# montyhall/bot7

Measured on AMD Instinct MI355X. Metric: EI candidates scored/sec at N=2048,d=32, higher is better.
Workload: dtype f64

## Files before the change

### bot7_amd/build.py

```python
import concurrent.futures
import os
import subprocess
import sys

HERE = os.path.dirname(os.path.abspath(__file__))
ROOT = os.path.dirname(HERE)
CSRC = os.path.join(HERE, "csrc")
BUILD = os.path.join(HERE, "_build")
OUT = os.path.join(HERE, "libbot7hip.so")
SOURCES = ["context.hip", "grid_api.hip", "gp_api.hip", "nominate.hip", "blr_api.hip", "sobol.hip", "covar.hip", "potrf.hip", "potrf_persist.hip", "posterior.hip", "score.hip", "extras.hip", "comm.hip", "group.hip", "blr_small.hip", "gp_small.hip", "kpost_small.hip", "batch.hip"]
DIAG_ONLY_SOURCES = ["nll_small.hip"]
DIAG_OUT = os.path.join(ROOT, "tools", "_build", "libbot7hip_diag.so")
HEADERS = [os.path.join(CSRC, "b7_internal.h"), os.path.join(CSRC, "gemm_f64.h"), os.path.join(CSRC, "potrf_diag.h"), os.path.join(CSRC, "comm_rccl.h"), os.path.join(CSRC, "ksx_exp.h"), os.path.join(CSRC, "exp_table.h"),
           os.path.join(ROOT, "include", "bot7hip.h")]
HIPCC = os.environ.get("HIPCC", "/opt/rocm/bin/hipcc")
FLAGS = ["-O3", "-std=c++17", "-fPIC", "--offload-arch=gfx950", "-fno-fast-math", "-Wall",
         "-I" + os.path.join(ROOT, "include"), "-I" + CSRC, "-I/opt/rocm/include"]


def _stale(target, deps):
    if not os.path.exists(target):
        return True
    t = os.path.getmtime(target)
    return any(os.path.getmtime(d) > t for d in deps)


EXTRA_FLAGS = {"covar.hip": ["-mllvm", "-amdgpu-mfma-vgpr-form"], "batch.hip": ["-mllvm", "-amdgpu-mfma-vgpr-form"]}


def _compile(src, diag=False):
    obj = os.path.join(BUILD, ("diag_" if diag else "") + src.replace(".hip", ".o"))
    path = os.path.join(CSRC, src)
    if _stale(obj, [path] + HEADERS + [os.path.abspath(__file__)]):
        subprocess.check_call([HIPCC] + FLAGS + EXTRA_FLAGS.get(src, []) + (["-DB7_DIAG"] if diag else []) + ["-c", path, "-o", obj])
        return obj, True
    return obj, False


def _mentions_diag(src):
    return "B7_DIAG" in open(os.path.join(CSRC, src)).read()


def build_diag(verbose=False):
    build()
    os.makedirs(os.path.dirname(DIAG_OUT), exist_ok=True)
    todo = [s for s in SOURCES if _mentions_diag(s)] + DIAG_ONLY_SOURCES
    with concurrent.futures.ThreadPoolExecutor(max_workers=min(8, len(todo))) as ex:
        res = dict(zip(todo, ex.map(lambda s: _compile(s, True), todo)))
    objs = [res[s][0] if s in res else os.path.join(BUILD, s.replace(".hip", ".o")) for s in SOURCES + DIAG_ONLY_SOURCES]
    if any(ch for _, ch in res.values()) or _stale(DIAG_OUT, objs):
        subprocess.check_call([HIPCC, "-shared", "-fPIC", "--offload-arch=gfx950", "-o", DIAG_OUT] + objs +
                              ["-ldl", "-Wl,-rpath,/opt/rocm/lib", "-Wl,--no-undefined", "-Wl,-Bsymbolic"])
        if verbose:
            print("built", DIAG_OUT)
    return DIAG_OUT


def posterior_isa():
    out = os.path.join(BUILD, "posterior.s")
    path = os.path.join(CSRC, "posterior.hip")
    if _stale(out, [path] + HEADERS + [os.path.abspath(__file__)]):
        subprocess.check_call([HIPCC] + [f for f in FLAGS if f != "-fPIC"] + ["-S", "--cuda-device-only", "-Wno-unused-command-line-argument",
                                                                            path, "-o", out])
    return out


def check_agpr_discipline():
    import re
    text = open(posterior_isa()).read()
    found = {}
    for m in re.finditer(r"^(_ZN\S*post_kernel_w4(?:ILi(\d)E|tILi\d+ELi\d+E)\S*):[^\n]*\n(.*?)\n\s*s_endpgm", text, flags=re.S | re.M):
        nj = int(m.group(2)) if m.group(2) else 16
        ntiles = 32 if nj == 16 else 8 * nj
        in_asm, stats, bad = False, {"mfma": 0, "mfma_from_zero": 0, "acc_reads": 0, "scratch": 0}, []
        for line in m.group(3).split("\n"):
            code = line.split(";")[0]
            if "ASMSTART" in line:
                in_asm = True
                continue
            if "ASMEND" in line:
                in_asm = False
                continue
            if in_asm:
                stats["mfma"] += "v_mfma_f64_16x16x4_f64" in code
                stats["mfma_from_zero"] += bool(re.search(r"v_mfma_f64_16x16x4_f64 a\[[^\]]*\], v\[[^\]]*\], v\[[^\]]*\], 0\s*$", code))
                stats["acc_reads"] += "v_accvgpr_read_b32" in code
            else:
                if re.search(r"(?<![A-Za-z0-9_.])a(\[|\d)", code):
                    bad.append(line.strip())
                stats["scratch"] += "scratch_" in code
        if bad or stats["scratch"] or stats["mfma_from_zero"] != ntiles or stats["acc_reads"] != 8 * ntiles:
            raise RuntimeError("post_kernel_w4<%d>: AGPR discipline broken: %r, compiler-generated AGPR uses: %r"
                               % (nj, stats, bad[:5]))
        found[nj] = stats
    if not {2, 4} <= set(found):
        raise RuntimeError("post_kernel_w4<2> and <4> expected in the ISA of posterior.hip, found %r" % sorted(found))
    return found


def build_post_probe():
    src = os.path.join(ROOT, "tools", "post_probe.hip")
    out = os.path.join(ROOT, "tools", "_build", "post_probe")
    os.makedirs(os.path.dirname(out), exist_ok=True)
    if _stale(out, [src, os.path.join(ROOT, "tools", "post_kernel_w8.h"), os.path.join(CSRC, "posterior.hip")] + HEADERS):
        subprocess.check_call([HIPCC, "--offload-arch=gfx950", "-O3", "-std=c++17", "-fno-fast-math", "-Wno-unused-value",
                               "-DB7_POST_NO_LAUNCHERS", "-I" + os.path.join(ROOT, "include"), "-I" + CSRC,
                               "-I/opt/rocm/include", "-o", out, src, "-Wl,-rpath,/opt/rocm/lib"])
    return out


def build(force=False, verbose=False):
    os.makedirs(BUILD, exist_ok=True)
    if force:
        for f in os.listdir(BUILD):
            os.remove(os.path.join(BUILD, f))
    with concurrent.futures.ThreadPoolExecutor(max_workers=min(8, len(SOURCES) + 2)) as ex:
        isa = ex.submit(check_agpr_discipline)
        probe = ex.submit(build_post_probe)
        results = list(ex.map(_compile, SOURCES))
        isa.result()
        probe.result()
    objs = [o for o, _ in results]
    if any(changed for _, changed in results) or _stale(OUT, objs):
        subprocess.check_call([HIPCC, "-shared", "-fPIC", "--offload-arch=gfx950", "-o", OUT] + objs +
                              ["-ldl", "-Wl,-rpath,/opt/rocm/lib", "-Wl,--no-undefined", "-Wl,-Bsymbolic"])
        if verbose:
            print("built", OUT)
    return OUT


if __name__ == "__main__":
    build(force="--force" in sys.argv, verbose=True)
    if "--diag" in sys.argv:
        build_diag(verbose=True)
```

### bot7_amd/csrc/b7_internal.h

```cpp
#pragma once
#include <hip/hip_runtime.h>
#include <stddef.h>
#include <stdint.h>

#include <map>
#include <string>
#include <vector>

#include "bot7hip.h"

constexpr int B7_NPAD = 128;
constexpr int B7_PANEL = 64;
constexpr int B7_PERSIST_NMAX = 4096;
constexpr int B7_MROWS = 256;
constexpr int B7_MAX_D = 96;

constexpr int B7_TAB_VAL = 0;
constexpr int B7_TAB_IDX = 1;
constexpr int B7_TAB_STATUS = 2;
constexpr int B7_TAB_ROWS = 3;
constexpr int B7_TAB_ROW0 = 4;
constexpr int B7_TAB_W = B7_TAB_ROW0 + B7_MAX_D;
constexpr int B7_MAX_WORLD = 64;

static inline int b7_dpad_class(int d) {
  return d <= 4 ? 4 : d <= 8 ? 8 : d <= 16 ? 16 : d <= 32 ? 32 : d <= 48 ? 48 : d <= 64 ? 64 : 96;
}

constexpr size_t B7_INFO_HEAD_BYTES = 16 + sizeof(double) * 257 + 8;
constexpr size_t B7_PERSIST_FLAG_WORDS_MAX = 16 + 2 * 64 * 64 + 2 * 64;
constexpr size_t B7_INFO_BYTES = B7_INFO_HEAD_BYTES + 4 * B7_PERSIST_FLAG_WORDS_MAX;

struct DevBuf {
  void *p = nullptr;
  size_t cap = 0;
};

struct PinBuf {
  void *host = nullptr, *dev = nullptr;
  size_t bytes = 0;
};

struct FitBlock { int info[4]; double terms[257]; };
struct BestPair { double v; int64_t i; };
constexpr int SOBOL_DIMS = 40;
constexpr int SOBOL_BITS = 30;
struct SobolTable {
  uint32_t v[SOBOL_DIMS][SOBOL_BITS];
};

constexpr size_t B7_PINNED_BYTES = 16384;
struct PinnedBlock {
  FitBlock fit;
  alignas(256) BestPair best;
  alignas(4096) double fmin[256];
  alignas(4096) double vec[B7_MAX_D + 3];
};
static_assert(offsetof(PinnedBlock, fit) == 0 && offsetof(PinnedBlock, best) == 2304 && offsetof(PinnedBlock, fmin) == 4096 &&
                  offsetof(PinnedBlock, vec) == 8192 && sizeof(PinnedBlock) <= B7_PINNED_BYTES,
              "pinned block: kernels and copies address these slots");

constexpr size_t B7_SCRATCH_BYTES = 64 * 1024;
struct ScratchBlock {
  double lenscale[256];
  double fmin[256];
  SobolTable sobol;
  double minmax[2 * B7_MAX_D];
  alignas(4096) double colvec[2 * B7_MAX_D];
};
static_assert(offsetof(ScratchBlock, lenscale) == 0 && offsetof(ScratchBlock, fmin) == 2048 && offsetof(ScratchBlock, sobol) == 4096 &&
                  offsetof(ScratchBlock, minmax) == 4096 + sizeof(SobolTable) && offsetof(ScratchBlock, colvec) == 12288 &&
                  sizeof(ScratchBlock) <= B7_SCRATCH_BYTES,
              "scratch block: the layout every earlier build used");

constexpr int B7_ACC_NONE = 0, B7_ACC_LINEAR = 1, B7_ACC_LOG = 2;

struct PhaseStat {
  double ms = 0.0;
  int64_t launches = 0;
};

struct ScoreParams {
  int kind = 0, S = 0, upper = 0;
  const double *mu = nullptr, *var = nullptr, *fmin = nullptr;
  long long stride = 0;
  double fmin0 = 0.0, tradeoff = 0.0, sign = 0.0;
};

struct b7_ctx {
  int device = 0;
  hipStream_t stream = nullptr;
  hipEvent_t ev_fit = nullptr;
  std::string err;
  int cus = 0;

  DevBuf grid[2];
  int grid_cur = 0;
  int64_t M = 0;
  int d = 0;

  bool fitted = false;
  bool have_data = false;
  int model_kind = 0;
  int N = 0, Npad = 0, dfit = 0, dpad = 0, ycols = 0;
  int yld = 1;
  double amp = 0, noise = 0, mean = 0;
  b7_gp_opts opts;
  int kernel = B7_KERNEL_ARDSE;
  DevBuf xobs;
  DevBuf w;
  DevBuf zsc;
  DevBuf zss;
  DevBuf K;
  DevBuf L;
  DevBuf Linv;
  DevBuf W;
  DevBuf dinv;
  DevBuf alpha;
  DevBuf resid;
  DevBuf atmp;
  DevBuf info;
  DevBuf ybuf;

  bool predicted = false;
  int64_t Mpred = 0;
  DevBuf mu;
  DevBuf var;
  DevBuf acc;
  bool acc_valid = false;
  int spin_us = 500;
  bool npad_small = true;
  bool potrf_small = true;
  bool blr_small = true;
  double fmin_scalar = 0.0;
  bool acc_fresh = false;
  int acc_kind = 0;
  DevBuf ks;
  size_t ks_bytes = (size_t)4 << 30;
  int diag_variant = 1;
  int inverse_inline = 1;
  PinnedBlock *pinned = nullptr, *pinned_dev = nullptr;
  std::vector<double> net_host;
  PinBuf pin_blr;
  PinBuf pin_eval;
  PinBuf pin_nll;
  bool fmin_staged = false;
  bool potrf_attrs_set = false;
  bool linv_done = false;
  int potrf_sched = 3;
  int syrk_small = 1;
  int potrf_defer = 1;
  int potrf_group = 2;
  struct JobList { DevBuf buf; int n = 0; };
  std::map<int, JobList> pjobs_cache;
  DevBuf pstamps;
  int pjobs_nb = 0, pjobs_n = 0;
  DevBuf bhyp, bw, bzsc, bzss, bK, bL, bdinv, bflags, binfo, bresid, bterms, bLinv, balpha, bmu, bvar;
  bool persist_attr_set = false, persist_stamps = false;
  int persist_helpers = 0;
  int persist_aborts = 0;
  int nll_small = 1;
  bool kpost_small = true;
  bool fit_small = true;
  int persist_fault = -1;
  int potrf_sched_saved = 0;
  DevBuf part;
  DevBuf ticket;
  DevBuf scratch;
  DevBuf tmpgrid;
  DevBuf tmpmu, tmpvar;
  DevBuf fant;
  DevBuf bel;
  DevBuf belvec;
  PinBuf pin_bel;
  DevBuf feat;
  size_t feat_zeroed_bytes = 0;
  int feat_z = -1;
  int64_t Mfeat = 0;
  int zdim = 0;
  uint64_t feat_version = 0, grid_version = 0;
  DevBuf netbuf;

  void *comm = nullptr;
  int comm_rank = 0, comm_world = 1;
  DevBuf slots;
  uint64_t *tab_host = nullptr;
  uint64_t *tab_host_dev = nullptr;
  struct b7_group *group = nullptr;
  bool group_busy = false;
  bool win_valid = false;
  int64_t win_idx1 = 0;
  int win_rank = -1, win_d = 0;
  double win_row[B7_MAX_D];
  int64_t shard_rows[B7_MAX_WORLD];
  int shard_world = 0;

  hipEvent_t tev[B7_MAX_TIMERS][2];
  bool tev_init = false;
  bool profile = false;
  std::map<std::string, PhaseStat> phases;
  struct PendingPhase { const char *name; hipEvent_t e0, e1; };
  std::vector<PendingPhase> pending;
  std::vector<hipEvent_t> free_events;
  hipEvent_t phase_e0 = nullptr;
};

int b7_fail(b7_ctx *c, int code, const char *fmt, ...);
#define B7_HIP(c, expr)                                                                          \
  do {                                                                                           \
    hipError_t e__ = (expr);                                                                     \
    if (e__ != hipSuccess)                                                                       \
      return b7_fail((c), e__ == hipErrorOutOfMemory ? B7_ERR_NOMEM : B7_ERR_HIP, "%s:%d: %s", \
                     __FILE_NAME__, __LINE__, hipGetErrorString(e__));                           \
  } while (0)
#define B7_TRY(expr)          \
  do {                        \
    int rc__ = (expr);        \
    if (rc__ != B7_OK) return rc__; \
  } while (0)

int b7_ensure(b7_ctx *c, DevBuf &b, size_t bytes);
void b7_release(DevBuf &b);
int b7_pin_ensure(b7_ctx *c, PinBuf &b, size_t bytes, bool mapped);
static inline ScratchBlock *b7_scratch(const b7_ctx *c) { return static_cast<ScratchBlock *>(c->scratch.p); }

struct PhaseScope {
  b7_ctx *c;
  const char *name;
  PhaseScope(b7_ctx *c, const char *name);
  ~PhaseScope();
};

static inline int64_t round_up(int64_t x, int64_t m) { return (x + m - 1) / m * m; }
int npad_of(const b7_ctx *c, int64_t n);

int launch_sobol(b7_ctx *c, double *out, int64_t size, int dims, int64_t skip, const double *mins,
                 const double *maxes);
int launch_random_grid(b7_ctx *c, double *out, int64_t size, int dims, uint64_t seed, int64_t row_offset,
                       const double *mins, const double *maxes);
int launch_remove_row(b7_ctx *c, const double *src, double *dst, int64_t M, int d, int64_t idx0);
int launch_remove_rows(b7_ctx *c, const double *src, double *dst, int64_t M, int d, const int64_t *cuts_dev, int ncut);
int launch_colrange(b7_ctx *c, const double *grid, int64_t M, int d, double *out_dev);
int launch_col_affine(b7_ctx *c, double *grid, int64_t M, int d, const double *v_dev, bool mul);
int launch_gather_rows(b7_ctx *c, const double *src, double *out, const int64_t *idx0_dev, int64_t n, int d);

struct KBatchDesc {
  int64_t s_w = 0, s_zsc = 0, s_zsh = 0, s_out = 0;
  const double *amp = nullptr;
  int64_t s_alpha = 0, s_mu = 0;
  const double *mean = nullptr;
};
struct ObsSet {
  const double *zsc;
  const double *zsh;
  int npad;
  const double *w = nullptr;
  KBatchDesc batch;
};
int launch_prep_obs_aux(b7_ctx *c, const double *xobs, const double *ls_dev, int N, int npad, double *zsc,
                        double *zsh);
int launch_k_generic(b7_ctx *c, const double *xq, int64_t rows, int64_t Mtotal, const ObsSet &o, double *out);
int launch_prep_obs(b7_ctx *c, const double *xobs, const double *lenscale_sq_dev, int N, int d);
int launch_kxx(b7_ctx *c, double diag_add);
int launch_ksx_batch(b7_ctx *c, int S, const double *xq, int64_t rows, int64_t Mtotal, const double *w, const double *zsc,
                     const double *zss, const double *amp_dev, const double *mean_dev, const double *alpha, double *ks,
                     int64_t s_out, double *mu, int64_t s_mu);
int launch_kxx_batch(b7_ctx *c, int B, const double *ls_dev, const double *amp_dev, const double *noise_dev, double *w,
                     double *zsc, double *zss, double *K);
int launch_ksx(b7_ctx *c, const double *xq, int64_t row0, int64_t rows, int64_t Mtotal, int d, double *ks,
               double *mu, int ycols);

struct FactorNote {
  bool alpha_done = false;
  int *report_written = nullptr;
};
int launch_potrf(b7_ctx *c, double extra, bool with_inverse, int *report_hint = nullptr, FactorNote *note = nullptr);
int launch_trtri(b7_ctx *c);
int launch_potrf_persist(b7_ctx *c, double extra, bool with_inverse);
int launch_nll_batch(b7_ctx *c, int B, const double *K, double *L, double *dinv, unsigned *flags, int *info,
                     const double *resid, double *terms);
int launch_nll_one(b7_ctx *c, const double *K, double *L, double *dinv, unsigned *flags, int *info, const double *resid,
                   double *terms, double extra);
size_t persist_flag_words_host(int nb);
int launch_potrf_small(b7_ctx *c, int B, const double *K, double *L, double *Linv, double *dinv, const double *resid, double *alpha,
                       double extra, int *info, int *report_dev, int64_t sK, int64_t sL, int64_t sdinv, int64_t svec, int sinfo);
int launch_blr_head_small(b7_ctx *c, const double *Z, int N, int z, int ldz, const double *yv, double alpha_prec, double beta,
                          int *report_dev);
int launch_blr_heads_small(b7_ctx *c, int S, const double *Z, int N, int z, int ldz, const double *yraw_dev, const double *hyp3_dev,
                           double *L, double *Linv, double *m, double *b, int *info, int *report_dev, double *terms);
int launch_post_heads(b7_ctx *c, int S, const double *Linv, const double *feat, int64_t rows, int64_t Mtotal, double *var, int64_t svar,
                      const double *zero_dev, const double *invbeta_dev);
int launch_gemv_rows_batch(b7_ctx *c, int S, const double *A, int lda, const double *x, int64_t sx, int n, const double *base_dev,
                           int64_t rows, double *y, int64_t sy);
int launch_nll_small(b7_ctx *c, int B, const double *hyp_dev, const double *hyp_host, double *terms_dev, int *info_dev,
                     unsigned *done_dev);
bool kpost_small_applies(const b7_ctx *c);
int launch_kpost_small(b7_ctx *c, int S, const double *xq, int64_t M, const double *w, const double *zsc, const double *zss,
                       const double *Linv, const double *alpha, const double *hyp_dev, double amp, double noise, double mean,
                       double *mu, double *var, int64_t sout);
bool gp_small_applies(const b7_ctx *c);
static inline bool fit_small_applies(const b7_ctx *c) {
  return c->fit_small && c->potrf_sched == 3 && c->inverse_inline && gp_small_applies(c);
}
int launch_nll_small8(b7_ctx *c, int B, const double *hyp_dev, const double *hyp_host, double *terms_dev, int *info_dev,
                      unsigned *done_dev);
int launch_fit_small(b7_ctx *c, int B, const double *hyp_dev, const double *hyp_host, double *hyp_out, double *w, double *zsc,
                     double *zss, double *L, double *Linv, double *dinv, double *alpha, double *resid, int *info_dev,
                     int *report_dev);
int launch_alpha(b7_ctx *c, int *report_dev = nullptr, int report_words = 0, const FactorNote &note = FactorNote());
int launch_alpha_batch(b7_ctx *c, int B, const double *Linv, const double *resid, double *alpha, const int *report_src = nullptr,
                       int *report_dev = nullptr, int report_words = 0);
int launch_fit_batch(b7_ctx *c, int B, const double *K, double *L, double *Linv, double *dinv, unsigned *flags, int *info);
int launch_nll_terms(b7_ctx *c, double *out_dev);
int launch_fro_norm_sq(b7_ctx *c, const double *A, int n, int ld, double *out_dev);
int launch_set_identity(b7_ctx *c);

// ... 137 lines not shown
```

### bot7_amd/csrc/context.hip

```cpp
#include <stdarg.h>
#include <stdio.h>
#include <stdlib.h>
#include <string.h>

#include "b7_internal.h"

static thread_local std::string g_create_err;

int b7_fail(b7_ctx *c, int code, const char *fmt, ...) {
  char buf[512];
  va_list ap;
  va_start(ap, fmt);
  vsnprintf(buf, sizeof(buf), fmt, ap);
  va_end(ap);
  if (c)
    c->err = buf;
  else
    g_create_err = buf;
  return code;
}

int b7_ensure(b7_ctx *c, DevBuf &b, size_t bytes) {
  if (bytes == 0) bytes = 16;
  if (b.cap >= bytes) return B7_OK;
  if (b.p) {
    B7_HIP(c, hipStreamSynchronize(c->stream));
    B7_HIP(c, hipFree(b.p));
    b.p = nullptr;
    b.cap = 0;
  }
  hipError_t e = hipMalloc(&b.p, bytes);
  if (e != hipSuccess) {
    b.p = nullptr;
    return b7_fail(c, B7_ERR_NOMEM, "hipMalloc(%zu bytes): %s", bytes, hipGetErrorString(e));
  }
  b.cap = bytes;
  return B7_OK;
}

void b7_release(DevBuf &b) {
  if (b.p) (void)hipFree(b.p);
  b.p = nullptr;
  b.cap = 0;
}

int b7_pin_ensure(b7_ctx *c, PinBuf &b, size_t bytes, bool mapped) {
  if (b.bytes >= bytes) return B7_OK;
  B7_HIP(c, hipStreamSynchronize(c->stream));
  if (b.host) (void)hipHostFree(b.host);
  b = PinBuf();
  B7_HIP(c, hipHostMalloc(&b.host, 2 * bytes, mapped ? hipHostMallocMapped : hipHostMallocDefault));
  if (mapped) B7_HIP(c, hipHostGetDevicePointer(&b.dev, b.host, 0));
  b.bytes = 2 * bytes;
  return B7_OK;
}

static hipEvent_t phase_event(b7_ctx *c) {
  if (!c->free_events.empty()) {
    hipEvent_t e = c->free_events.back();
    c->free_events.pop_back();
    return e;
  }
  hipEvent_t e = nullptr;
  (void)hipEventCreate(&e);
  return e;
}

static void resolve_phases(b7_ctx *c) {
  if (c->pending.empty()) return;
  (void)hipStreamSynchronize(c->stream);
  for (const b7_ctx::PendingPhase &p : c->pending) {
    float ms = 0.f;
    if (p.e0 && p.e1 && hipEventElapsedTime(&ms, p.e0, p.e1) == hipSuccess) {
      PhaseStat &s = c->phases[p.name];
      s.ms += ms;
      s.launches += 1;
    }
    if (p.e0) c->free_events.push_back(p.e0);
    if (p.e1) c->free_events.push_back(p.e1);
  }
  c->pending.clear();
}

PhaseScope::PhaseScope(b7_ctx *c_, const char *name_) : c(c_), name(name_) {
  if (!c->profile) return;
  c->phase_e0 = phase_event(c);
  if (c->phase_e0) (void)hipEventRecord(c->phase_e0, c->stream);
}
PhaseScope::~PhaseScope() {
  if (!c->profile || !c->phase_e0) return;
  hipEvent_t e1 = phase_event(c);
  if (e1) (void)hipEventRecord(e1, c->stream);
  c->pending.push_back({name, c->phase_e0, e1});
  c->phase_e0 = nullptr;
  if (c->pending.size() >= 4096) resolve_phases(c);
}

int npad_of(const b7_ctx *c, int64_t n) { return (c->npad_small && n <= 64) ? 64 : (int)round_up(n, B7_NPAD); }

static int timers_init(b7_ctx *c) {
  if (c->tev_init) return B7_OK;
  for (int i = 0; i < B7_MAX_TIMERS; ++i) {
    B7_HIP(c, hipEventCreate(&c->tev[i][0]));
    B7_HIP(c, hipEventCreate(&c->tev[i][1]));
  }
  c->tev_init = true;
  return B7_OK;
}

extern "C" {

int b7_abi_version(void) { return B7_ABI_VERSION; }

int b7_create(b7_ctx **out, int device_id) {
  if (!out) return b7_fail(nullptr, B7_ERR_INVALID, "b7_create: out is NULL");
  *out = nullptr;
  int ndev = 0;
  hipError_t e = hipGetDeviceCount(&ndev);
  if (e != hipSuccess || ndev <= 0)
    return b7_fail(nullptr, B7_ERR_HIP, "no HIP device available (%s); libbot7hip has no CPU path",
                   e == hipSuccess ? "device count 0" : hipGetErrorString(e));
  if (device_id < 0 || device_id >= ndev)
    return b7_fail(nullptr, B7_ERR_INVALID, "device_id %d out of range [0,%d)", device_id, ndev);
  e = hipSetDevice(device_id);
  if (e != hipSuccess) return b7_fail(nullptr, B7_ERR_HIP, "hipSetDevice: %s", hipGetErrorString(e));
  hipDeviceProp_t prop;
  e = hipGetDeviceProperties(&prop, device_id);
  if (e != hipSuccess) return b7_fail(nullptr, B7_ERR_HIP, "hipGetDeviceProperties: %s", hipGetErrorString(e));
  if (strncmp(prop.gcnArchName, "gfx950", 6) != 0)
    return b7_fail(nullptr, B7_ERR_UNSUPPORTED, "device %d is %s; libbot7hip is built for gfx950 only", device_id,
                   prop.gcnArchName);
  b7_ctx *c = new b7_ctx();
  c->device = device_id;
  c->cus = prop.multiProcessorCount;
  b7_gp_default_opts(&c->opts);
  if (const char *pv = getenv("B7_SPIN_US")) c->spin_us = atoi(pv);
#ifdef B7_DIAG
  if (const char *pv = getenv("B7_DIAG_VARIANT")) c->diag_variant = atoi(pv);
  if (const char *pv = getenv("B7_NPAD_SMALL")) c->npad_small = atoi(pv) != 0;
  if (const char *pv = getenv("B7_POTRF_SMALL")) c->potrf_small = atoi(pv) != 0;
  if (getenv("B7_POTRF_SCHED") || getenv("B7_DIAG_VARIANT") || getenv("B7_INVERSE_INLINE")) c->potrf_small = c->fit_small = false;
  if (const char *pv = getenv("B7_BLR_SMALL")) c->blr_small = atoi(pv) != 0;
  if (const char *pv = getenv("B7_INVERSE_INLINE")) c->inverse_inline = atoi(pv);
  if (const char *pv = getenv("B7_POTRF_SCHED")) c->potrf_sched = atoi(pv);
  c->persist_stamps = getenv("B7_PERSIST_STAMPS") != nullptr;
  if (const char *pv = getenv("B7_PERSIST_HELPERS")) c->persist_helpers = atoi(pv);
  if (const char *pv = getenv("B7_PERSIST_FAULT")) c->persist_fault = atoi(pv);
  if (const char *pv = getenv("B7_NLL_SMALL")) c->nll_small = atoi(pv);
  if (const char *pv = getenv("B7_FIT_SMALL")) c->fit_small = atoi(pv) != 0;
  if (const char *pv = getenv("B7_KPOST_SMALL")) c->kpost_small = atoi(pv) != 0;
  if (const char *pv = getenv("B7_SYRK_SMALL")) c->syrk_small = atoi(pv) ? 1 : 0;
  if (const char *pv = getenv("B7_POTRF_DEFER")) c->potrf_defer = atoi(pv) ? 1 : 0;
  if (const char *pv = getenv("B7_POTRF_GROUP")) {
    const int g = atoi(pv);
    if (g >= 1 && g <= 8) c->potrf_group = g;
  }
#endif
  e = hipStreamCreateWithFlags(&c->stream, hipStreamNonBlocking);
  if (e == hipSuccess) e = hipEventCreateWithFlags(&c->ev_fit, hipEventDisableTiming);
  if (e == hipSuccess) e = hipHostMalloc((void **)&c->pinned, B7_PINNED_BYTES, hipHostMallocMapped);
  if (e == hipSuccess) e = hipHostGetDevicePointer((void **)&c->pinned_dev, c->pinned, 0);
  if (e != hipSuccess) {
    if (c->pinned) (void)hipHostFree(c->pinned);
    if (c->stream) (void)hipStreamDestroy(c->stream);
    delete c;
    return b7_fail(nullptr, B7_ERR_HIP, "stream / pinned result block creation: %s", hipGetErrorString(e));
  }
  if (b7_ensure(c, c->scratch, B7_SCRATCH_BYTES) != B7_OK) {
    g_create_err = c->err;
    b7_destroy(c);
    return B7_ERR_NOMEM;
  }
  *out = c;
  return B7_OK;
}

void b7_destroy(b7_ctx *c) {
  if (!c) return;
  (void)hipSetDevice(c->device);
  (void)hipStreamSynchronize(c->stream);
  (void)b7_comm_destroy(c);
  DevBuf *all[] = {&c->grid[0], &c->grid[1], &c->xobs, &c->w,     &c->zsc,  &c->zss,     &c->K,      &c->L,
                   &c->Linv,    &c->W,       &c->dinv, &c->alpha, &c->resid, &c->info,   &c->ybuf,   &c->mu,
                   &c->var,     &c->acc,     &c->ks,   &c->part,  &c->scratch, &c->tmpgrid, &c->tmpmu, &c->tmpvar, &c->fant, &c->feat, &c->netbuf, &c->atmp, &c->slots, &c->pstamps,
                   &c->bhyp, &c->bw, &c->bzsc, &c->bzss, &c->bK, &c->bL, &c->bdinv, &c->bflags, &c->binfo, &c->bresid, &c->bterms,
                   &c->bLinv, &c->balpha, &c->bmu, &c->bvar, &c->ticket, &c->bel, &c->belvec};
  for (auto &kv : c->pjobs_cache) b7_release(kv.second.buf);
  for (DevBuf *b : all) b7_release(*b);
  if (c->tev_init)
    for (int i = 0; i < B7_MAX_TIMERS; ++i) {
      (void)hipEventDestroy(c->tev[i][0]);
      (void)hipEventDestroy(c->tev[i][1]);
    }
  resolve_phases(c);
  if (c->pinned) (void)hipHostFree(c->pinned);
  for (PinBuf *b : {&c->pin_eval, &c->pin_blr, &c->pin_nll, &c->pin_bel})
    if (b->host) (void)hipHostFree(b->host);
  if (c->tab_host) (void)hipHostFree(c->tab_host);
  for (hipEvent_t e : c->free_events) (void)hipEventDestroy(e);
  if (c->phase_e0) (void)hipEventDestroy(c->phase_e0);
  if (c->ev_fit) (void)hipEventDestroy(c->ev_fit);
  (void)hipStreamDestroy(c->stream);
  delete c;
}

const char *b7_last_error(const b7_ctx *c) { return c ? c->err.c_str() : g_create_err.c_str(); }

int b7_device_info(b7_ctx *c, char *name_out, int *compute_units, int64_t *hbm_bytes) {
  if (!c) return B7_ERR_INVALID;
  hipDeviceProp_t prop;
  B7_HIP(c, hipGetDeviceProperties(&prop, c->device));
  if (name_out) snprintf(name_out, 64, "%s (%s)", prop.name, prop.gcnArchName);
  if (compute_units) *compute_units = prop.multiProcessorCount;
  if (hbm_bytes) *hbm_bytes = (int64_t)prop.totalGlobalMem;
  return B7_OK;
}

int b7_sync(b7_ctx *c) {
  if (!c) return B7_ERR_INVALID;
  B7_HIP(c, hipStreamSynchronize(c->stream));
  return B7_OK;
}

int b7_set_workspace(b7_ctx *c, int64_t bytes) {
  if (!c || bytes < (int64_t)(8 * 128 * 128)) return c ? b7_fail(c, B7_ERR_INVALID, "workspace too small") : B7_ERR_INVALID;
  c->ks_bytes = (size_t)bytes;
  return B7_OK;
}

int b7_timer_start(b7_ctx *c, int slot) {
  if (!c || slot < 0 || slot >= B7_MAX_TIMERS) return B7_ERR_INVALID;
  B7_TRY(timers_init(c));
  B7_HIP(c, hipEventRecord(c->tev[slot][0], c->stream));
  return B7_OK;
}

int b7_timer_stop(b7_ctx *c, int slot) {
  if (!c || slot < 0 || slot >= B7_MAX_TIMERS) return B7_ERR_INVALID;
  B7_TRY(timers_init(c));
  B7_HIP(c, hipEventRecord(c->tev[slot][1], c->stream));
  return B7_OK;
}

int b7_timer_ms(b7_ctx *c, int slot, float *ms_out) {
  if (!c || slot < 0 || slot >= B7_MAX_TIMERS || !ms_out) return B7_ERR_INVALID;
  B7_TRY(timers_init(c));
  B7_HIP(c, hipEventSynchronize(c->tev[slot][1]));
  B7_HIP(c, hipEventElapsedTime(ms_out, c->tev[slot][0], c->tev[slot][1]));
  return B7_OK;
}

int b7_profile_enable(b7_ctx *c, int on) {
  if (!c) return B7_ERR_INVALID;
  c->profile = on != 0;
  return B7_OK;
}

int b7_profile_reset(b7_ctx *c) {
  if (!c) return B7_ERR_INVALID;
  resolve_phases(c);
  c->phases.clear();
  return B7_OK;
}

int b7_profile_get(b7_ctx *c, const char *phase, double *ms_total, int64_t *launches) {
  if (!c || !phase) return B7_ERR_INVALID;
  resolve_phases(c);
  auto it = c->phases.find(phase);
  if (ms_total) *ms_total = it == c->phases.end() ? 0.0 : it->second.ms;
  if (launches) *launches = it == c->phases.end() ? 0 : it->second.launches;
  return B7_OK;
}

}
```

### bot7_amd/csrc/posterior.hip

```cpp
#include "b7_internal.h"
#include <utility>

#ifdef B7_POST_STAMPS
__device__ unsigned long long b7_post_stamps[4 * 4096];
extern "C" int b7dbg_post_stamps(unsigned long long *out, int nblocks) {
  return (int)hipMemcpyFromSymbol(out, HIP_SYMBOL(b7_post_stamps), sizeof(unsigned long long) * 4 * nblocks);
}
#endif

typedef double d2_t __attribute__((ext_vector_type(2)));

struct PostBatch {
  int64_t sLinv = 0, sks = 0, svar = 0;
  const double *base = nullptr, *var_add = nullptr;
};

namespace w4 {
constexpr int BM = 128, BK = 16, LD = BK + 1, A_DBL = BM * LD;

#define B7_W4_ACC_REGS \
  "a0", "a1", "a2", "a3", "a4", "a5", "a6", "a7", "a8", "a9", "a10", "a11", "a12", "a13", "a14", "a15", \
  "a16", "a17", "a18", "a19", "a20", "a21", "a22", "a23", "a24", "a25", "a26", "a27", "a28", "a29", "a30", \
  "a31", "a32", "a33", "a34", "a35", "a36", "a37", "a38", "a39", "a40", "a41", "a42", "a43", "a44", "a45", \
  "a46", "a47", "a48", "a49", "a50", "a51", "a52", "a53", "a54", "a55", "a56", "a57", "a58", "a59", "a60", \
// ... 292 lines not shown
      mfma_tile<NJ, i, j, ZERO>(use.a[i], use.b[j]);
      static_for<KMAX>([&](auto k_) {
        constexpr int sidx = m * NSIDE / NM + decltype(k_)::value;
        if constexpr (sidx < (m + 1) * NSIDE / NM) side(std::integral_constant<int, sidx>{});
      });
    });
  }

  template <int FIRST, int NEXT_FIRST, bool ZERO>
  static __device__ __forceinline__ void stage(Set &s0, Set &s1, Data &g, double *__restrict__ cur, double *__restrict__ nxt,
                                               int fa, int fb, int wofs, const double *__restrict__ pa,
                                               const double *__restrict__ pb, int64_t lda, Cursor &ld) {
    constexpr int H = NC / 2;
    const double *qa = pa + ((int64_t)ld.t * BMT) * lda + ld.kb * BK, *qb = pb + ld.kb * BK;
    ld.advance();
    kstep<FIRST, ZERO, NP + H>(s0, [&](auto s_) {
      constexpr int x = decltype(s_)::value;
      if constexpr (x < NP) {
        if constexpr (x < NJ || x - NJ >= FIRST) read_one<x, 1>(s1, cur + fa, cur + fb);
      } else {
        store_chunk<x - NP>(g, nxt + wofs);
      }
    });
    kstep<FIRST, false, NP + NC - H>(s1, [&](auto s_) {
      constexpr int x = decltype(s_)::value;
      if constexpr (x < NP) {
        if constexpr (x < NJ || x - NJ >= FIRST) read_one<x, 2>(s0, cur + fa, cur + fb);
      } else {
        store_chunk<H + x - NP>(g, nxt + wofs);
      }
    });
    kstep<FIRST, false, NP + NC>(s0, [&](auto s_) {
      constexpr int x = decltype(s_)::value;
      if constexpr (x < NP) {
        if constexpr (x < NJ || x - NJ >= FIRST) read_one<x, 3>(s1, cur + fa, cur + fb);
      } else {
        load_chunk<x - NP>(g, qa, qb, lda);
      }
    });
    __builtin_amdgcn_s_waitcnt(0xC07F);
    __builtin_amdgcn_s_barrier();
    kstep<FIRST, false, NP>(s1, [&](auto s_) {
      constexpr int x = decltype(s_)::value;
      if constexpr (x < NJ || x - NJ >= NEXT_FIRST) read_one<x, 0>(s0, nxt + fa, nxt + fb);
    });
  }
};

template <int NJ, int NR>
__global__ void __launch_bounds__(256)
    post_kernel_w4t(const double *__restrict__ Linv, const double *__restrict__ ks, int Npad, int64_t row0, int64_t Mtotal,
                    double base, double sgn, double var_add, int clamp, double var_min, double *__restrict__ var,
                    PostBatch bat) {
  using T = Tall<NJ, NR>;
  constexpr int BMT = T::BMT, BN = T::BN, NC = T::NC, NP = T::NP;
  extern __shared__ __align__(16) double sm[];
  if (bat.base) {
    const int64_t y = blockIdx.y;
    Linv += y * bat.sLinv;
    ks += y * bat.sks;
    var += y * bat.svar;
    base = bat.base[y];
    if (bat.var_add) var_add = bat.var_add[y];
  }
  const int lane = threadIdx.x & 63, wave = __builtin_amdgcn_readfirstlane(threadIdx.x >> 6);
#ifdef B7_POST_STAMPS
  const unsigned long long st0 = __builtin_amdgcn_s_memtime(), sr0 = __builtin_amdgcn_s_memrealtime();
  __builtin_amdgcn_s_waitcnt(0xC07F);
#endif
  const int64_t lda = Npad;
  const int r0 = threadIdx.x >> 3, kc = threadIdx.x & 7;
  const double *pa = Linv + (int64_t)r0 * lda + 2 * kc;
  const double *pb = ks + ((int64_t)blockIdx.x * BN + r0) * lda + 2 * kc;
  const int wofs = r0 * LD + 2 * kc;
  const int fa = (lane & 15) * LD + (lane >> 4);
  const int fb = T::A_DBLT + (wave * 16 * NJ + (lane & 15)) * LD + (lane >> 4);

  const int ntiles = Npad / BMT;
  typename T::Cursor ld{0, 0, ntiles};
  typename T::Data g;
  typename T::Set s0, s1;
  double *const b0 = sm, *const b1 = sm + T::STAGE_DBL;
  static_for<NC>([&](auto c_) { T::template load_chunk<decltype(c_)::value>(g, pa, pb, lda); });
  ld.advance();
  static_for<NC>([&](auto c_) { T::template store_chunk<decltype(c_)::value>(g, b0 + wofs); });
  {
    const double *qa = pa + ((int64_t)ld.t * BMT) * lda + ld.kb * BK, *qb = pb + ld.kb * BK;
    static_for<NC>([&](auto c_) { T::template load_chunk<decltype(c_)::value>(g, qa, qb, lda); });
    ld.advance();
  }
  __builtin_amdgcn_s_waitcnt(0xC07F);
  __builtin_amdgcn_s_barrier();
  static_for<NP>([&](auto p_) { T::template read_one<decltype(p_)::value, 0>(s0, b0 + fa, b0 + fb); });

  double colss[2][NJ] = {};
#define B7_STAGE(F, NF, Z, CUR, NXT) T::template stage<F, NF, Z>(s0, s1, g, CUR, NXT, fa, fb, wofs, pa, pb, lda, ld)
  for (int t = 0; t < ntiles; ++t) {
    B7_STAGE(0, 0, true, b0, b1);
    if (t > 0) {
      for (int p = 0; p < (NR / 2) * t - 1; ++p) {
        B7_STAGE(0, 0, false, b1, b0);
        B7_STAGE(0, 0, false, b0, b1);
      }
      B7_STAGE(0, 0, false, b1, b0);
      B7_STAGE(0, 1, false, b0, b1);
    }
    static_for<NR - 1>([&](auto q_) {
      constexpr int Q = decltype(q_)::value + 1;
      if constexpr (Q % 2 == 1)
        B7_STAGE(Q, (Q + 1) % NR, false, b1, b0);
      else
        B7_STAGE(Q, (Q + 1) % NR, false, b0, b1);
    });
    asm volatile("s_nop 15\n\ts_nop 15\n\ts_nop 15" ::: "memory");
    static_for<(NR / 4) * NJ>([&](auto qj_) {
      constexpr int q = decltype(qj_)::value / NJ, j = decltype(qj_)::value % NJ;
      double s = 0.0;
      static_for<4>([&](auto i_) {
        double v[4];
        read_tile<NJ, 4 * q + decltype(i_)::value, j>(v);
#pragma unroll
        for (int r = 0; r < 4; ++r) s = __builtin_fma(v[r], v[r], s);
      });
      colss[q & 1][j] += s;
    });
  }
#undef B7_STAGE

#pragma unroll
  for (int j = 0; j < NJ; ++j) {
    double v0 = colss[0][j], v1 = colss[1][j];
    v0 += __shfl_xor(v0, 16);
    v0 += __shfl_xor(v0, 32);
    v1 += __shfl_xor(v1, 16);
    v1 += __shfl_xor(v1, 32);
    const int64_t gidx = row0 + (int64_t)blockIdx.x * BN + wave * 16 * NJ + j * 16 + lane;
    if (lane < 16 && gidx < Mtotal) {
      double ss = v0;
      ss += v1;
      double v = (base + sgn * ss) + var_add;
      if (clamp) v = (v < var_min) ? var_min : v;
      var[gidx] = v;
    }
  }
#ifdef B7_POST_STAMPS
  if (threadIdx.x == 0 && blockIdx.x < 4096) {
    const unsigned long long st1 = __builtin_amdgcn_s_memtime(), sr1 = __builtin_amdgcn_s_memrealtime();
    __builtin_amdgcn_s_waitcnt(0xC07F);
    unsigned long long *o = b7_post_stamps + 4 * blockIdx.x;
    o[0] = st0, o[1] = sr0, o[2] = st1, o[3] = sr1;
  }
#endif
}
}

namespace small64 {
typedef double d4_t __attribute__((ext_vector_type(4)));
constexpr int NB = 64, LLD = NB + 2, BN = 64;
constexpr int LDS_BYTES = BN * LLD * 8;

__global__ void __launch_bounds__(256)
    post_small_kernel(const double *__restrict__ Linv, const double *__restrict__ ks, int64_t row0, int64_t Mtotal, int ntiles,
                      double base, double sgn, double var_add, int clamp, double var_min, double *__restrict__ var, PostBatch bat) {
  extern __shared__ __align__(16) double sm[];
  if (bat.base) {
    const int64_t y = blockIdx.y;
    Linv += y * bat.sLinv;
    ks += y * bat.sks;
    var += y * bat.svar;
    base = bat.base[y];
    if (bat.var_add) var_add = bat.var_add[y];
  }
  double *Ks = sm;
  const int tid = threadIdx.x, lane = tid & 63, wave = tid >> 6, lr = lane & 15, lq = lane >> 4;
  d2_t pv[BN / 8];
  auto fetch = [&](int tile) {
    const double *kt = ks + ((int64_t)tile * BN) * NB;
#pragma unroll
    for (int i = 0; i < BN / 8; ++i) {
      const int e = tid + 256 * i;
      pv[i] = *reinterpret_cast<const d2_t *>(kt + (int64_t)(e >> 5) * NB + 2 * (e & 31));
    }
  };
  int tile = blockIdx.x;
  if (tile < ntiles) fetch(tile);
  double af[40];
#pragma unroll
  for (int I = 0; I < 4; ++I)
#pragma unroll
    for (int k4 = 0; k4 < 4 * (I + 1); ++k4) af[2 * I * (I + 1) + k4] = Linv[(int64_t)(I * 16 + lr) * NB + 4 * k4 + lq];
#pragma unroll
  for (int g = 0; g < 4; ++g)
    asm volatile("" : "+v"(af[10 * g]), "+v"(af[10 * g + 1]), "+v"(af[10 * g + 2]), "+v"(af[10 * g + 3]), "+v"(af[10 * g + 4]),
                      "+v"(af[10 * g + 5]), "+v"(af[10 * g + 6]), "+v"(af[10 * g + 7]), "+v"(af[10 * g + 8]), "+v"(af[10 * g + 9]));
  for (; tile < ntiles; tile += gridDim.x) {
#pragma unroll
    for (int i = 0; i < BN / 8; ++i) {
      const int e = tid + 256 * i, r = e >> 5, c2 = 2 * (e & 31);
      Ks[r * LLD + c2] = pv[i][0];
      Ks[r * LLD + c2 + 1] = pv[i][1];
    }
    __syncthreads();
    if (tile + (int)gridDim.x < ntiles) fetch(tile + gridDim.x);
    __builtin_amdgcn_sched_barrier(0);
    constexpr int NJ = BN / 64;
    double ss[NJ];
#pragma unroll
    for (int j = 0; j < NJ; ++j) {
      const double *bp = Ks + (wave * 16 * NJ + j * 16 + lr) * LLD + lq;
      double bf[16];
#pragma unroll
      for (int k4 = 0; k4 < 16; ++k4) bf[k4] = bp[4 * k4];
      double s = 0.0;
#pragma unroll
      for (int I = 0; I < 4; ++I) {
        d4_t c = {0.0, 0.0, 0.0, 0.0};
#ifdef B7_PS_ABLATE
        c = __builtin_amdgcn_mfma_f64_16x16x4f64(af[2 * I * (I + 1)], bf[I], c, 0, 0, 0);
#else
#pragma unroll
        for (int k4 = 0; k4 < 4 * (I + 1); ++k4) c = __builtin_amdgcn_mfma_f64_16x16x4f64(af[2 * I * (I + 1) + k4], bf[k4], c, 0, 0, 0);
#endif
#pragma unroll
        for (int r = 0; r < 4; ++r) s = __builtin_fma(c[r], c[r], s);
      }
      ss[j] = s;
    }
#pragma unroll
    for (int j = 0; j < NJ; ++j) {
      double v = ss[j];
      v += __shfl_xor(v, 16);
      v += __shfl_xor(v, 32);
      const int64_t gidx = row0 + (int64_t)tile * BN + wave * 16 * NJ + j * 16 + lr;
      if (lane < 16 && gidx < Mtotal) {
        double o = (base + sgn * v) + var_add;
        if (clamp) o = (o < var_min) ? var_min : o;
        var[gidx] = o;
      }
    }
    __syncthreads();
  }
}
}

#ifndef B7_POST_NO_LAUNCHERS
namespace {
struct PostArgs {
  const double *Linv, *ks;
  double *var;
  double base, sgn, var_add;
  int S;
  PostBatch pb;
};

template <int NJ>
int launch_post_w4(b7_ctx *c, const PostArgs &a, int64_t row0, int64_t rows, int64_t Mtotal) {
  constexpr int lds = w4::lds_bytes<NJ>();
  B7_HIP(c, hipFuncSetAttribute(reinterpret_cast<const void *>(w4::post_kernel_w4<NJ>),
                                hipFuncAttributeMaxDynamicSharedMemorySize, lds));
  hipLaunchKernelGGL(w4::post_kernel_w4<NJ>, dim3((unsigned)(rows / (64 * NJ)), a.S), dim3(256), lds, c->stream, a.Linv, a.ks,
                     c->Npad, row0, Mtotal, a.base, a.sgn, a.var_add, c->opts.var_clamp, c->opts.var_min, a.var, a.pb);
  B7_HIP(c, hipGetLastError());
  return B7_OK;
}

template <int NJ, int NR>
int launch_post_tall(b7_ctx *c, const PostArgs &a, int64_t row0, int64_t rows, int64_t Mtotal) {
  using T = w4::Tall<NJ, NR>;
  auto kern = w4::post_kernel_w4t<NJ, NR>;
  B7_HIP(c, hipFuncSetAttribute(reinterpret_cast<const void *>(kern), hipFuncAttributeMaxDynamicSharedMemorySize,
                                T::LDS_BYTES));
  hipLaunchKernelGGL(kern, dim3((unsigned)(rows / T::BN), a.S), dim3(256), T::LDS_BYTES, c->stream, a.Linv, a.ks, c->Npad, row0,
                     Mtotal, a.base, a.sgn, a.var_add, c->opts.var_clamp, c->opts.var_min, a.var, a.pb);
  B7_HIP(c, hipGetLastError());
  return B7_OK;
}

int launch_post_small(b7_ctx *c, const PostArgs &a, int64_t row0, int64_t rows, int64_t Mtotal) {
  B7_HIP(c, hipFuncSetAttribute(reinterpret_cast<const void *>(small64::post_small_kernel), hipFuncAttributeMaxDynamicSharedMemorySize,
                                small64::LDS_BYTES));
  const int ntiles = (int)(rows / small64::BN), S = a.S > 0 ? a.S : 1;
  int gx = (2 * c->cus + S - 1) / S;
  if (gx > ntiles) gx = ntiles;
  if (gx < 1) gx = 1;
  hipLaunchKernelGGL(small64::post_small_kernel, dim3((unsigned)gx, S), dim3(256), small64::LDS_BYTES, c->stream, a.Linv, a.ks, row0,
                     Mtotal, ntiles, a.base, a.sgn, a.var_add, c->opts.var_clamp, c->opts.var_min, a.var, a.pb);
  B7_HIP(c, hipGetLastError());
  return B7_OK;
}

int dispatch_post(b7_ctx *c, const PostArgs &a, int64_t row0, int64_t rows, int64_t Mtotal) {
  if (rows % B7_MROWS) return b7_fail(c, B7_ERR_INVALID, "post: rows %lld not a multiple of %d", (long long)rows, B7_MROWS);
  if (c->Npad == 64) return launch_post_small(c, a, row0, rows, Mtotal);
  const bool large = rows / 256 * a.S >= c->cus;
  if (c->Npad % 256 == 0 && large) return launch_post_tall<2, 16>(c, a, row0, rows, Mtotal);
  if (!large) return launch_post_w4<2>(c, a, row0, rows, Mtotal);
  return launch_post_w4<4>(c, a, row0, rows, Mtotal);
}
}

int launch_post(b7_ctx *c, const double *ks, int64_t row0, int64_t rows, int64_t Mtotal, double *var) {
  PhaseScope ps(c, "post");
  const bool blr = c->model_kind == 1;
  PostArgs a{(const double *)c->Linv.p, ks, var, blr ? 0.0 : c->amp, blr ? 1.0 : -1.0,
             blr ? c->noise : (c->opts.var_with_noise ? c->noise : 0.0), 1, PostBatch{}};
  return dispatch_post(c, a, row0, rows, Mtotal);
}

int launch_post_batch(b7_ctx *c, int S, const double *Linv, const double *ks, int64_t sks, int64_t rows, int64_t Mtotal,
                      double *var, int64_t svar, const double *amp_dev, const double *noise_dev) {
  PhaseScope ps(c, "post");
  PostArgs a{Linv, ks, var, 0.0, -1.0, 0.0, S, PostBatch{}};
  a.pb.sLinv = (int64_t)c->Npad * c->Npad;
  a.pb.sks = sks;
  a.pb.svar = svar;
  a.pb.base = amp_dev;
  a.pb.var_add = c->opts.var_with_noise ? noise_dev : nullptr;
  return dispatch_post(c, a, 0, rows, Mtotal);
}

int launch_post_heads(b7_ctx *c, int S, const double *Linv, const double *feat, int64_t rows, int64_t Mtotal, double *var, int64_t svar,
                      const double *zero_dev, const double *invbeta_dev) {
  PhaseScope ps(c, "post");
  PostArgs a{Linv, feat, var, 0.0, 1.0, 0.0, S, PostBatch{}};
  a.pb.sLinv = (int64_t)c->Npad * c->Npad;
  a.pb.sks = 0;
  a.pb.svar = svar;
  a.pb.base = zero_dev;
  a.pb.var_add = invbeta_dev;
  return dispatch_post(c, a, 0, rows, Mtotal);
}
#endif
```

Measured before the change: 16.18 million.

## Add direct-load tall posterior kernel with register-prefetched B and LDS-staged A

Adds a new tall posterior variance kernel (post_kernel_w4d) in which each wave loads its ks (B) fragments straight from global memory into registers, double-buffered across two k-halves. The Linv (A) panels are staged through double-buffered LDS, with the global-to-LDS copies interleaved into the MFMA k-steps. It becomes the default for large, 256-aligned Npad cases, replacing launch_post_tall<2,16>; diagnostic builds can still select the older variants. The aim is to cut LDS traffic and hide load latency behind MFMA work, at the cost of more VGPR pressure and a more intricate schedule.

Result: no change. 16.11 million (-0.4%).

```diff
diff --git a/bot7_amd/build.py b/bot7_amd/build.py
--- a/bot7_amd/build.py
+++ b/bot7_amd/build.py
@@ -69,7 +69,7 @@
     import re
     text = open(posterior_isa()).read()
     found = {}
-    for m in re.finditer(r"^(_ZN\S*post_kernel_w4(?:ILi(\d)E|tILi\d+ELi\d+E)\S*):[^\n]*\n(.*?)\n\s*s_endpgm", text, flags=re.S | re.M):
+    for m in re.finditer(r"^(_ZN\S*post_kernel_w4(?:ILi(\d)E|tILi\d+ELi\d+E|dILi\d+ELi\d+ELi\d+E)\S*):[^\n]*\n(.*?)\n\s*s_endpgm", text, flags=re.S | re.M):
         nj = int(m.group(2)) if m.group(2) else 16
         ntiles = 32 if nj == 16 else 8 * nj
         in_asm, stats, bad = False, {"mfma": 0, "mfma_from_zero": 0, "acc_reads": 0, "scratch": 0}, []
@@ -93,8 +93,8 @@
             raise RuntimeError("post_kernel_w4<%d>: AGPR discipline broken: %r, compiler-generated AGPR uses: %r"
                                % (nj, stats, bad[:5]))
         found[nj] = stats
-    if not {2, 4} <= set(found):
-        raise RuntimeError("post_kernel_w4<2> and <4> expected in the ISA of posterior.hip, found %r" % sorted(found))
+    if not {2, 4, 16} <= set(found):
+        raise RuntimeError("post_kernel_w4<2>, <4> and the tall shape expected in the ISA of posterior.hip, found %r" % sorted(found))
     return found
 
 
diff --git a/bot7_amd/csrc/b7_internal.h b/bot7_amd/csrc/b7_internal.h
--- a/bot7_amd/csrc/b7_internal.h
+++ b/bot7_amd/csrc/b7_internal.h
@@ -162,6 +162,7 @@
   int nll_small = 1;
   bool kpost_small = true;
   bool fit_small = true;
+  int post_tall = 0;
   int persist_fault = -1;
   int potrf_sched_saved = 0;
   DevBuf part;
diff --git a/bot7_amd/csrc/context.hip b/bot7_amd/csrc/context.hip
--- a/bot7_amd/csrc/context.hip
+++ b/bot7_amd/csrc/context.hip
@@ -149,6 +149,7 @@
   if (const char *pv = getenv("B7_NLL_SMALL")) c->nll_small = atoi(pv);
   if (const char *pv = getenv("B7_FIT_SMALL")) c->fit_small = atoi(pv) != 0;
   if (const char *pv = getenv("B7_KPOST_SMALL")) c->kpost_small = atoi(pv) != 0;
+  if (const char *pv = getenv("B7_POST_TALL")) c->post_tall = atoi(pv);
   if (const char *pv = getenv("B7_SYRK_SMALL")) c->syrk_small = atoi(pv) ? 1 : 0;
   if (const char *pv = getenv("B7_POTRF_DEFER")) c->potrf_defer = atoi(pv) ? 1 : 0;
   if (const char *pv = getenv("B7_POTRF_GROUP")) {
diff --git a/bot7_amd/csrc/posterior.hip b/bot7_amd/csrc/posterior.hip
--- a/bot7_amd/csrc/posterior.hip
+++ b/bot7_amd/csrc/posterior.hip
@@ -468,6 +468,223 @@
   }
 #endif
 }
+
+template <int NJ, int NR, int BKD>
+struct TallD {
+  static constexpr int BMT = 16 * NR, BN = 64 * NJ, LDD = BKD + 1, STAGE_DBL = BMT * LDD, KS = BKD / 4;
+  static constexpr int CPR = BKD / 2, RPP = 256 / CPR, NCA = BMT / RPP;
+  static constexpr int HS = BMT / BKD;
+  static constexpr int LDS_BYTES = 2 * STAGE_DBL * 8;
+  static_assert(NJ * NR == 32, "32 accumulator tiles per wave");
+  static_assert(BKD == 16 || BKD == 32, "a stage is one or two 16-deep halves");
+
+  struct Set {
+    double a[NR];
+  };
+  struct Data {
+    d2_t c[NCA];
+  };
+  struct Cursor {
+    int t, kb, ntiles;
+    __device__ __forceinline__ void advance() {
+      if (kb + 1 < (t + 1) * HS) {
+        ++kb;
+      } else if (t + 1 < ntiles) {
+        ++t;
+        kb = 0;
+      }
+    }
+  };
+
+  template <int C>
+  static __device__ __forceinline__ void load_chunk(Data &g, const double *__restrict__ qa, int64_t lda) {
+    g.c[C] = *reinterpret_cast<const d2_t *>(qa + (int64_t)(RPP * C) * lda);
+  }
+  template <int C>
+  static __device__ __forceinline__ void store_chunk(const Data &g, double *w) {
+    auto *o = (__attribute__((address_space(3))) volatile double *)(w + RPP * C * LDD);
+    o[0] = g.c[C][0];
+    o[1] = g.c[C][1];
+  }
+  template <int H>
+  static __device__ __forceinline__ void load_half(double (&bf)[2][4][NJ], const double *__restrict__ qb, int64_t lda) {
+    static_for<4 * NJ>([&](auto x_) {
+      constexpr int s = decltype(x_)::value / NJ, j = decltype(x_)::value % NJ;
+      bf[H][s][j] = qb[(int64_t)(16 * j) * lda + 4 * s];
+    });
+  }
+
+  template <int FIRST, bool ZERO, int NSIDE, class Side, class Reload>
+  static __device__ __forceinline__ void kstep(const Set &use, const double (&b)[NJ], bool skip_first, Side &&side, Reload &&reload) {
+    constexpr int NI = NR - FIRST, NM = NJ * NI;
+    constexpr int KMAX = (NSIDE + NM - 1) / NM + 1;
+    static_for<NM>([&](auto m_) {
+      constexpr int m = decltype(m_)::value, i = FIRST + m / NJ, j = m % NJ;
+      if (i > FIRST || !skip_first) mfma_tile<NJ, i, j, ZERO>(use.a[i], b[j]);
+      static_for<KMAX>([&](auto k_) {
+        constexpr int sidx = m * NSIDE / NM + decltype(k_)::value;
+        if constexpr (sidx < (m + 1) * NSIDE / NM) side(std::integral_constant<int, sidx>{});
+      });
+      if constexpr (m >= NM - NJ) reload(std::integral_constant<int, j>{});
+    });
+  }
+
+  template <int F0, int F1, int NF, bool ZERO, int PAR>
+  static __device__ __forceinline__ void stage(Set &s0, Set &s1, Data &g, double (&bf)[2][4][NJ], double *__restrict__ b0,
+                                               double *__restrict__ b1, int fa, int wofs, const double *__restrict__ pa,
+                                               const double *__restrict__ pbf, int64_t lda, Cursor &ld, Cursor &lb,
+                                               bool skip1 = false) {
+    double *cur = PAR ? b1 : b0, *nxt = PAR ? b0 : b1;
+    const double *qa = pa + ((int64_t)ld.t * BMT) * lda + ld.kb * BKD, *qb = pbf + lb.kb * BKD;
+    ld.advance();
+    lb.advance();
+    static_for<KS>([&](auto s_) {
+      constexpr int s = decltype(s_)::value, FIRST = s < 4 ? F0 : F1, FNEXT = s + 1 == KS ? NF : (s + 1 < 4 ? F0 : F1);
+      constexpr int H = BKD == 16 ? PAR : s / 4;
+      constexpr int NST = s < KS / 2 ? NCA / (KS / 2) : 0, ST0 = s * NST;
+      constexpr int NLK = KS / 2 - 1, u = s - KS / 2;
+      constexpr int LD0 = (u >= 0 && u < NLK) ? u * NCA / NLK : 0, NLD = (u >= 0 && u < NLK) ? (u + 1) * NCA / NLK - LD0 : 0;
+      const Set &use = s % 2 ? s1 : s0;
+      Set &fill = s % 2 ? s0 : s1;
+      const double *src = (s + 1 == KS ? nxt : cur) + fa + 4 * ((s + 1) % KS);
+      if constexpr (s + 1 == KS) {
+        __builtin_amdgcn_s_waitcnt(0xC07F);
+        __builtin_amdgcn_s_barrier();
+      }
+      kstep<FIRST, ZERO && s == 0, NR + NST + NLD>(
+          use, bf[H][s % 4], s >= 4 && skip1,
+          [&](auto x_) {
+            constexpr int x = decltype(x_)::value;
+            if constexpr (x < NR) {
+              if constexpr (x >= FNEXT) fill.a[x] = src[x * 16 * LDD];
+            } else if constexpr (x < NR + NST) {
+              store_chunk<ST0 + x - NR>(g, nxt + wofs);
+            } else {
+              load_chunk<LD0 + x - NR - NST>(g, qa, lda);
+            }
+          },
+          [&](auto j_) {
+            constexpr int j = decltype(j_)::value;
+            bf[H][s % 4][j] = qb[(int64_t)(16 * j) * lda + 4 * s];
+          });
+    });
+  }
+};
+
+template <int NJ, int NR, int BKD>
+__global__ void __launch_bounds__(256)
+    post_kernel_w4d(const double *__restrict__ Linv, const double *__restrict__ ks, int Npad, int64_t row0, int64_t Mtotal,
+                    double base, double sgn, double var_add, int clamp, double var_min, double *__restrict__ var,
+                    PostBatch bat) {
+  using T = TallD<NJ, NR, BKD>;
+  constexpr int BMT = T::BMT, BN = T::BN, NCA = T::NCA, HS = T::HS;
+  extern __shared__ __align__(16) double sm[];
+  if (bat.base) {
+    const int64_t y = blockIdx.y;
+    Linv += y * bat.sLinv;
+    ks += y * bat.sks;
+    var += y * bat.svar;
+    base = bat.base[y];
+    if (bat.var_add) var_add = bat.var_add[y];
+  }
+  const int lane = threadIdx.x & 63, wave = __builtin_amdgcn_readfirstlane(threadIdx.x >> 6);
+#ifdef B7_POST_STAMPS
+  const unsigned long long st0 = __builtin_amdgcn_s_memtime(), sr0 = __builtin_amdgcn_s_memrealtime();
+  __builtin_amdgcn_s_waitcnt(0xC07F);
+#endif
+  const int64_t lda = Npad;
+  const int r0 = threadIdx.x / T::CPR, kc = threadIdx.x % T::CPR;
+  const double *pa = Linv + (int64_t)r0 * lda + 2 * kc;
+  const int wofs = r0 * T::LDD + 2 * kc;
+  const int fa = (lane & 15) * T::LDD + (lane >> 4);
+  const double *pbf = ks + ((int64_t)blockIdx.x * BN + wave * 16 * NJ + (lane & 15)) * lda + (lane >> 4);
+
+  const int ntiles = Npad / BMT;
+  typename T::Cursor ld{0, 0, ntiles}, lb{0, 0, ntiles};
+  typename T::Data g;
+  typename T::Set s0, s1;
+  double bf[2][4][NJ];
+  double *const b0 = sm, *const b1 = sm + T::STAGE_DBL;
+  static_for<NCA>([&](auto c_) { T::template load_chunk<decltype(c_)::value>(g, pa, lda); });
+  ld.advance();
+  if constexpr (BKD == 16) {
+    T::template load_half<0>(bf, pbf, lda);
+    lb.advance();
+    T::template load_half<1>(bf, pbf + lb.kb * BKD, lda);
+    lb.advance();
+  } else {
+    T::template load_half<0>(bf, pbf, lda);
+    T::template load_half<1>(bf, pbf + 16, lda);
+    lb.advance();
+  }
+  static_for<NCA>([&](auto c_) { T::template store_chunk<decltype(c_)::value>(g, b0 + wofs); });
+  {
+    const double *qa = pa + ((int64_t)ld.t * BMT) * lda + ld.kb * BKD;
+    static_for<NCA>([&](auto c_) { T::template load_chunk<decltype(c_)::value>(g, qa, lda); });
+    ld.advance();
+  }
+  __builtin_amdgcn_s_waitcnt(0xC07F);
+  __builtin_amdgcn_s_barrier();
+  static_for<NR>([&](auto p_) { s0.a[decltype(p_)::value] = b0[fa + decltype(p_)::value * 16 * T::LDD]; });
+
+  double colss[2][NJ] = {};
+#define B7_STAGE(F0, F1, NF, Z, PAR, ...) \
+  T::template stage<F0, F1, NF, Z, PAR>(s0, s1, g, bf, b0, b1, fa, wofs, pa, pbf, lda, ld, lb, ##__VA_ARGS__)
+  constexpr int D1 = BKD / 16, DF1 = D1 - 1;
+  for (int t = 0; t < ntiles; ++t) {
+    B7_STAGE(0, 0, 0, true, 0, DF1 && t == 0);
+    if (t > 0) {
+      for (int p = 0; p < (HS / 2) * t - 1; ++p) {
+        B7_STAGE(0, 0, 0, false, 1);
+        B7_STAGE(0, 0, 0, false, 0);
+      }
+      B7_STAGE(0, 0, 0, false, 1);
+      B7_STAGE(0, DF1, D1, false, 0);
+    }
+    static_for<HS - 1>([&](auto q_) {
+      constexpr int Q = decltype(q_)::value + 1, F0 = Q * D1;
+      B7_STAGE(F0, F0 + DF1, ((Q + 1) % HS) * D1, false, Q % 2);
+    });
+    asm volatile("s_nop 15\n\ts_nop 15\n\ts_nop 15" ::: "memory");
+    static_for<(NR / 4) * NJ>([&](auto qj_) {
+      constexpr int q = decltype(qj_)::value / NJ, j = decltype(qj_)::value % NJ;
+      double s = 0.0;
+      static_for<4>([&](auto i_) {
+        double v[4];
+        read_tile<NJ, 4 * q + decltype(i_)::value, j>(v);
+#pragma unroll
+        for (int r = 0; r < 4; ++r) s = __builtin_fma(v[r], v[r], s);
+      });
+      colss[q & 1][j] += s;
+    });
+  }
+#undef B7_STAGE
+
+#pragma unroll
+  for (int j = 0; j < NJ; ++j) {
+    double v0 = colss[0][j], v1 = colss[1][j];
+    v0 += __shfl_xor(v0, 16);
+    v0 += __shfl_xor(v0, 32);
+    v1 += __shfl_xor(v1, 16);
+    v1 += __shfl_xor(v1, 32);
+    const int64_t gidx = row0 + (int64_t)blockIdx.x * BN + wave * 16 * NJ + j * 16 + lane;
+    if (lane < 16 && gidx < Mtotal) {
+      double ss = v0;
+      ss += v1;
+      double v = (base + sgn * ss) + var_add;
+      if (clamp) v = (v < var_min) ? var_min : v;
+      var[gidx] = v;
+    }
+  }
+#ifdef B7_POST_STAMPS
+  if (threadIdx.x == 0 && blockIdx.x < 4096) {
+    const unsigned long long st1 = __builtin_amdgcn_s_memtime(), sr1 = __builtin_amdgcn_s_memrealtime();
+    __builtin_amdgcn_s_waitcnt(0xC07F);
+    unsigned long long *o = b7_post_stamps + 4 * blockIdx.x;
+    o[0] = st0, o[1] = sr0, o[2] = st1, o[3] = sr1;
+  }
+#endif
+}
 }
 
 namespace small64 {
@@ -592,6 +809,18 @@
   return B7_OK;
 }
 
+template <int NJ, int NR, int BKD>
+int launch_post_direct(b7_ctx *c, const PostArgs &a, int64_t row0, int64_t rows, int64_t Mtotal) {
+  using T = w4::TallD<NJ, NR, BKD>;
+  auto kern = w4::post_kernel_w4d<NJ, NR, BKD>;
+  B7_HIP(c, hipFuncSetAttribute(reinterpret_cast<const void *>(kern), hipFuncAttributeMaxDynamicSharedMemorySize,
+                                T::LDS_BYTES));
+  hipLaunchKernelGGL(kern, dim3((unsigned)(rows / T::BN), a.S), dim3(256), T::LDS_BYTES, c->stream, a.Linv, a.ks, c->Npad, row0,
+                     Mtotal, a.base, a.sgn, a.var_add, c->opts.var_clamp, c->opts.var_min, a.var, a.pb);
+  B7_HIP(c, hipGetLastError());
+  return B7_OK;
+}
+
 int launch_post_small(b7_ctx *c, const PostArgs &a, int64_t row0, int64_t rows, int64_t Mtotal) {
   B7_HIP(c, hipFuncSetAttribute(reinterpret_cast<const void *>(small64::post_small_kernel), hipFuncAttributeMaxDynamicSharedMemorySize,
                                 small64::LDS_BYTES));
@@ -609,7 +838,14 @@
   if (rows % B7_MROWS) return b7_fail(c, B7_ERR_INVALID, "post: rows %lld not a multiple of %d", (long long)rows, B7_MROWS);
   if (c->Npad == 64) return launch_post_small(c, a, row0, rows, Mtotal);
   const bool large = rows / 256 * a.S >= c->cus;
-  if (c->Npad % 256 == 0 && large) return launch_post_tall<2, 16>(c, a, row0, rows, Mtotal);
+  if (c->Npad % 256 == 0 && large) {
+#ifdef B7_DIAG
+    if (c->post_tall == 1) return launch_post_tall<2, 16>(c, a, row0, rows, Mtotal);
+    if (c->post_tall == 2) return launch_post_direct<2, 16, 16>(c, a, row0, rows, Mtotal);
+    if (c->post_tall == 3) return launch_post_w4<4>(c, a, row0, rows, Mtotal);
+#endif
+    return launch_post_direct<2, 16, 32>(c, a, row0, rows, Mtotal);
+  }
   if (!large) return launch_post_w4<2>(c, a, row0, rows, Mtotal);
   return launch_post_w4<4>(c, a, row0, rows, Mtotal);
 }
```
